# cartographer-project/cartographer

Measured on AMD Instinct MI355X. Metric: candidate poses scored/sec, higher is better.
Workload: dtype u8/int32; 1 GPU; C2: 2D FastCorrelativeScanMatcher MatchFullSubmap (branch and bound): 1000-point scan vs 1 400x400 submap(s) per GPU, depth 7, full-angle search, m...; submaps_per_gpu=1, rotations=2373, found=1

## Files before the change

### cartographer_amd/csrc/cmx_common.h

```cpp
#ifndef CMX_COMMON_H_
#define CMX_COMMON_H_

#include <hip/hip_runtime.h>

#include <cstdarg>
#include <cstdint>
#include <cstdio>
#include <cstring>
#include <functional>
#include <mutex>
#include <string>
#include <vector>

#include "../../include/cartographer_mi355x.h"

namespace cmx {

void SetLastError(const char* fmt, ...);
const char* LastError();

struct HipError {
  cmx_status status;
};

// ... 26 lines not shown
  } catch (const std::bad_alloc&) {
    SetLastError("host allocation failed");
    return CMX_OUT_OF_MEMORY;
  } catch (const std::exception& e) {
    SetLastError("exception: %s", e.what());
    return CMX_DEVICE_ERROR;
  }
}

#define CMX_DEBUG_OPTIONS(X)                                                                      \
  X(rt2d_legacy)                 \
  X(rt2d_tile)                                        \
  X(rt2d_groups)                                   \
  X(rt2d_target)                                    \
  X(rt2d_lds_kb)                                         \
  X(rt2d_no_image_cache)             \
  X(rt2d_parts)                                 \
  X(rt2d_host_par)         \
  X(rt2d_tables_serial)    \
  X(rt2d_first_part)       \
  X(rt2d_image_kernels)    \
  X(rt2d_no_lane)          \
  X(rt2d_parts_pool)       \
  X(rt2d_grid_share)       \
  X(rt2d_unfused)            \
  X(rt2d_no_bounds)        \
  X(rt2d_bounds)           \
  X(rt2d_bounds_fused)     \
  X(rt2d_bounds_level)     \
  X(rt2d_bounds_verify)    \
  X(rt2d_tsdf_batch_legacy)  \
  X(rt2d_tsdf_batch_bulk)  \
  X(rt2d_tsdf_verify)      \
  X(timeline)                  \
  X(trace)                       \
  X(host_trace)                          \
  X(launch_serial)         \
  X(sync)                      \
  X(no_copy_kernels)             \
  X(timing)                \
  X(no_direct_results)     \
  X(frontier_capacity)     \
  X(comm_virtual_ranks)    \
  X(comm_force_rccl)       \
  X(fast2d_unfused)                    \
  X(fast2d_store_scans)                   \
  X(fast2d_fused_threads)                            \
  X(fast2d_fanout)         \
  X(fast2d_group)          \
  X(fast2d_group_verify)   \
  X(fast2d_levels_per_stage)                                    \
  X(fast2d_wave_levels)                        \
  X(fast2d_xcd_affinity)                          \
  X(fast2d_queue)          \
  X(fast2d_queue_blocks)                \
  X(fast2d_queue_capacity)              \
  X(fast2d_queue_lost)       \
  X(filters_generic)       \
  X(fast3d_byte_loads)                             \
  X(fast3d_affinity)                              \
  X(fast3d_no_families)                             \
  X(fast3d_no_oct)                                         \
  X(fast3d_batch)                                                 \
  X(fast3d_chunk_cells)    \
  X(rt3d_legacy)                  \
  X(rt3d_no_tiles)                      \
  X(rt3d_verify)                  \
  X(rt3d_no_rotblocks)              \
  X(rt3d_rotblock_permille)  \
  X(rt3d_crosscheck)           \
  X(rt3d_expand_all)       \
  X(rt3d_unstaged)                                     \
  X(rt3d_no_boxes)                            \
  X(rt3d_report)                                             \
  X(rt3d_segments)                         \
  X(rt3d_group_rotations)                                  \
  X(rt3d_group_tile_kb)                                   \
  X(rt3d_group_float)                          \
  X(rt3d_cand_threads)                                   \
  X(rt3d_cand_rotations)                                    \
  X(rt3d_cand_tile_kb)
struct DebugOptions {
#define CMX_DEBUG_FIELD(name) int name = 0;
  CMX_DEBUG_OPTIONS(CMX_DEBUG_FIELD)
#undef CMX_DEBUG_FIELD
};
const DebugOptions& Debug();
bool DebugSet(const char* name, int value);

void UseDevice(int device);

void ParallelFor(int n, int serial_below, const std::function<void(int)>& fn);

class LaunchTurn {
 public:
  LaunchTurn();
  ~LaunchTurn();
  LaunchTurn(const LaunchTurn&) = delete;
  LaunchTurn& operator=(const LaunchTurn&) = delete;
 private:
  bool held_;
};

class HostLane {
 public:
  HostLane();
// ... 161 lines not shown
```

### cartographer_amd/csrc/fast_2d.hip

```cpp
#include <algorithm>
#include <chrono>
#include <cstring>
#include <memory>
#include <type_traits>
#include <utility>

#include "fast_2d_device.h"
#include "fast_2d_internal.h"

namespace cmx {
namespace {

constexpr int kSeedsPerProblem = 64;

constexpr int kMaxStages = kMaxDepth + 2;

constexpr int kCountStride = 32;
constexpr int kQueues = 2048;
struct alignas(8) QueueCtl {
  int head;
  int reserved;
  int pad[30];
};
struct Counters {
// ... 15 lines not shown
  int frontier_overflow;
  int leaf_overflow;
  unsigned wave_gathers;
  int pad;
  unsigned queue_stats[8];
};

struct NodeList {
  Node2D* nodes;
  int* counts;
  int sub_capacity;
};

__device__ __forceinline__ int ListReserve(const NodeList& list, int sub, int m) {
  return atomicAdd(&list.counts[sub * kCountStride], m);
}
__device__ __forceinline__ bool ListStore(const NodeList& list, int sub, int slot,
                                          const Node2D& nd) {
  if (slot >= list.sub_capacity) return false;
  list.nodes[static_cast<size_t>(sub) * list.sub_capacity + slot] = nd;
  return true;
}
__device__ __forceinline__ int ListMaxCount(const NodeList& list) {
  const int lane = threadIdx.x & 63;
  return WaveMax(min(list.counts[lane * kCountStride], list.sub_capacity));
}

__device__ __forceinline__ int NodeProblem(const Node2D& nd) { return nd.problem & 0xffffff; }
__device__ __forceinline__ int NodeLevel(const Node2D& nd) { return nd.problem >> 24; }

__device__ __forceinline__ Node2D CoarseNode(const Fast2DProblem& P, int problem, int s,
                                             int local) {
  const int2 dims = P.coarse_dims[s];
  const int4 bd = P.bounds[s];
  const int step = 1 << (P.depth - 1);
  const int ix = local / dims.y, iy = local - ix * dims.y;
  const int c = s * P.coarse_stride + local;
  Node2D nd;
  nd.problem = problem | ((P.depth - 1) << 24);
  nd.scan = s;
  nd.dx = bd.x + ix * step;
  nd.dy = bd.z + iy * step;
  nd.score = P.coarse_score[c];
  nd.coarse_index = c;
  nd.path = 0;
  nd.coarse_score = nd.score;
  return nd;
}

struct SeedScratch {
  int hist[1024];
  int wave_total[4];
  int threshold_bin;
  int found_scan;
  int total;
};

__device__ __forceinline__ bool PickSeed(const Fast2DProblem& P, int n, int want,
                                         SeedScratch* sh, int* scan_out) {
  const int tid = threadIdx.x, lane = tid & 63, T = blockDim.x;
  for (int i = tid; i < 1024; i += T) sh->hist[i] = 0;
  if (tid == 0) { sh->found_scan = -1; sh->total = 0; }
  __syncthreads();
  const int S = P.num_scans;
  const long long range = 255ll * n + 1;
  const auto* scan_best = AsGlobal(P.scan_best);
  const auto* coarse_dims = AsGlobal(P.coarse_dims);
  const bool grouped = P.group > 1;
  const auto best_of = [&](int s) -> int {
    if (grouped) {
      const int first = s - s % kFusedGroup;
      if (s != first + (S - first >= kFusedGroup ? 1 : 0)) return -1;
    }
    return scan_best[s].x;
  };
  constexpr int kOwn = 16;
  int own[kOwn];
#pragma unroll
  for (int k = 0; k < kOwn; ++k) {
    const int s = tid + k * T;
    own[k] = s < S ? best_of(s) : -1;
  }
  int total = 0;
#pragma unroll
  for (int k = 0; k < kOwn; ++k)
    if (own[k] >= 0) atomicAdd(&sh->hist[static_cast<int>(own[k] * 1024ll / range)], 1);
  for (int s = tid + kOwn * T; s < S; s += T) {
    const int b = best_of(s);
    if (b >= 0) atomicAdd(&sh->hist[static_cast<int>(b * 1024ll / range)], 1);
  }
  if (want == 0) {
    for (int s = tid; s < S; s += T) total += coarse_dims[s].x * coarse_dims[s].y;
    total = WaveSum(total);
    if (lane == 0 && total) atomicAdd(&sh->total, total);
  }
  __syncthreads();
  if (tid < 64) {
    int mine = 0;
#pragma unroll
    for (int k = 0; k < 16; ++k) mine += sh->hist[1023 - 16 * lane - k];
    int incl = mine;
#pragma unroll
    for (int off = 1; off < 64; off <<= 1) {
      const int o = __shfl_up(incl, off, 64);
      if (lane >= off) incl += o;
    }
    const unsigned long long reached = __ballot(incl >= kSeedsPerProblem);
    int tb = 0;
    if (reached) {
      const int first = __ffsll(static_cast<long long>(reached)) - 1;
      if (lane == first) {
        int acc = incl - mine;
        for (int k = 0; k < 16; ++k) {
          const int b = 1023 - 16 * lane - k;
          acc += sh->hist[b];
          if (acc >= kSeedsPerProblem) { tb = b; break; }
        }
        sh->threshold_bin = tb;
      }
    } else if (lane == 0) {
      sh->threshold_bin = 0;
    }
  }
  __syncthreads();
  const int tb = sh->threshold_bin;
  const auto qualifies = [&](int best) {
    return best >= 0 && static_cast<int>(best * 1024ll / range) >= tb &&
           ToScore(P, best, n) > P.min_score;
  };
  int count = 0;
#pragma unroll
  for (int k = 0; k < kOwn; ++k) count += qualifies(own[k]) ? 1 : 0;
  for (int s = tid + kOwn * T; s < S; s += T) count += qualifies(best_of(s)) ? 1 : 0;
  int incl = count;
#pragma unroll
  for (int off = 1; off < 64; off <<= 1) {
    const int o = __shfl_up(incl, off, 64);
    if (lane >= off) incl += o;
  }
  if (lane == 63) sh->wave_total[tid >> 6] = incl;
  __syncthreads();
  int before = incl - count;
  for (int w = 0; w < (tid >> 6); ++w) before += sh->wave_total[w];
  if (want >= before && want < before + count) {
    int k = before, found = -1;
#pragma unroll
    for (int j = 0; j < kOwn; ++j) {
      if (found < 0 && qualifies(own[j])) {
        if (k == want) found = tid + j * T;
        ++k;
      }
    }
    for (int s = tid + kOwn * T; s < S && found < 0; s += T) {
      if (!qualifies(best_of(s))) continue;
      if (k == want) found = s;
      ++k;
    }
    sh->found_scan = found;
  }
  __syncthreads();
  *scan_out = sh->found_scan;
  return sh->found_scan >= 0;
}

constexpr int kPointCache = 4096;

struct BlockContext {
  LevelDesc level[kMaxDepth];
  uint32_t cache[kPointCache];
  const uint32_t* global_pts;
  float min_s, score_scale, min_score;
  int n, cached;
  int max_x, max_y;
};

__device__ __forceinline__ void LoadContext(const Fast2DProblem& P, int n, int scan,
                                            BlockContext* ctx, bool stored = false) {
  const uint32_t* pts = P.discrete + static_cast<size_t>(scan) * n;
  const bool cached = n <= kPointCache;
  if (P.recompute_scans && !stored) {
    const float2 rot = P.scan_rot[scan];
    for (int i = threadIdx.x; i < n; i += blockDim.x) ctx->cache[i] = ScanCell(P, rot, i);
  } else if (cached) {
    const auto* gp = AsGlobal(pts);
    for (int i = threadIdx.x; i < n; i += blockDim.x) ctx->cache[i] = gp[i];
  }
  if (threadIdx.x < kMaxDepth && static_cast<int>(threadIdx.x) < P.depth)
    ctx->level[threadIdx.x] = P.level[threadIdx.x];
  if (threadIdx.x == 64) {
    const int4 bd = P.bounds[scan];
    ctx->max_x = bd.y;
    ctx->max_y = bd.w;
    ctx->global_pts = pts;
    ctx->cached = cached;
    ctx->n = n;
    ctx->min_s = P.min_s;
    ctx->score_scale = P.score_scale;
    ctx->min_score = P.min_score;
  }
  __syncthreads();
}

__device__ __forceinline__ float ToScoreCtx(const BlockContext& ctx, int sum) {
  return ctx.min_s + (static_cast<float>(sum) / static_cast<float>(ctx.n)) * ctx.score_scale;
}

struct ChildScratch {
  int partial[4][4];
  float child_score[4];
  int rank[4];
  int nvalid;
};

__device__ __forceinline__ void ScoreChildren(const BlockContext& ctx, int dx, int dy,
                                              int child_level, ChildScratch* sh) {
// ... 773 lines not shown
                                        int home, Node2D* out, unsigned* lost_races,
                                        unsigned* slot_rereads) {
  for (;;) {
    const unsigned long long hr =
        LoadAgent(reinterpret_cast<const unsigned long long*>(&counters->queue[home].head));
    const int head = static_cast<int>(hr & 0xffffffffu);
    const int reserved = min(static_cast<int>(hr >> 32), Q.capacity);
    if (reserved <= head) return false;
    if (TakeSlot(counters, home, head)) {
      ReadSlot(Q, home, head, out, slot_rereads);
      return true;
    }
    ++*lost_races;
  }
}

__device__ __forceinline__ bool Steal(const TreeQueue& Q, Counters* __restrict__ counters,
                                      int home, int queues, unsigned salt, int windows,
                                      int max_lost, Node2D* out, unsigned* lost_races,
                                      unsigned* slot_rereads) {
  const int lane = threadIdx.x & 63;
  int lost = 0;
  for (int w = 0; w < windows; ++w) {
    const int base = static_cast<int>((static_cast<unsigned>(home) * 2654435761u + salt * 40503u + w * 64u) %
                                      static_cast<unsigned>(queues));
    const int mine = (base + lane) % queues;
    const unsigned long long hr =
        LoadAgent(reinterpret_cast<const unsigned long long*>(&counters->queue[mine].head));
    const int head = static_cast<int>(hr & 0xffffffffu);
    const int reserved = min(static_cast<int>(hr >> 32), Q.capacity);
    const unsigned long long avail = __ballot(reserved > head);
    if (avail == 0) continue;
    int skip = static_cast<int>((salt + home) % static_cast<unsigned>(__popcll(avail)));
    unsigned long long rest = avail;
    while (skip-- > 0) rest &= rest - 1;
    const int l = __ffsll(static_cast<long long>(rest)) - 1;
    const int q = (base + l) % queues;
    const int slot = __builtin_amdgcn_readlane(head, l);
    if (TakeSlot(counters, q, slot)) {
      ReadSlot(Q, q, slot, out, slot_rereads);
      return true;
    }
    ++*lost_races;
    if (++lost >= max_lost) return false;
    --w;
    ++salt;
  }
  return false;
}

constexpr int kChainCells = 16;
constexpr uint32_t kNoCell = 0x80008000u;

__device__ __forceinline__ void RecordLeafAgent(const Node2D& leaf, const NodeList& leaves,
                                                int sub, Counters* __restrict__ counters) {
  const int slot = ListReserve(leaves, sub, 1);
  if (slot >= leaves.sub_capacity) {
    __hip_atomic_store(&counters->leaf_overflow, 1, __ATOMIC_RELAXED, __HIP_MEMORY_SCOPE_AGENT);
    return;
  }
  unsigned long long v[4];
  __builtin_memcpy(v, &leaf, sizeof(Node2D));
  unsigned long long* at = reinterpret_cast<unsigned long long*>(
      &leaves.nodes[static_cast<size_t>(sub) * leaves.sub_capacity + slot]);
#pragma unroll
  for (int k = 0; k < 4; ++k)
    __hip_atomic_store(&at[k], v[k], __ATOMIC_RELAXED, __HIP_MEMORY_SCOPE_AGENT);
}

__global__ void __launch_bounds__(256)
TreeQueueKernel(const Fast2DProblem* __restrict__ problems, ProblemState* __restrict__ states, int n,
                NodeList in, TreeQueue Q, NodeList leaves, Counters* __restrict__ counters,
                SelectState* __restrict__ sel, BestLeaf* __restrict__ best_out, int num_problems,
                ProblemState* __restrict__ states_out, CountersSummary* __restrict__ summary,
                const unsigned* __restrict__ tail_dev, unsigned* __restrict__ tail_host,
                int tail_words, int counters_trace, int max_lost) {
  static_assert(sizeof(Node2D) == 32, "a node is eight words: eight granules, four leaf stores");
  const int lane = threadIdx.x & 63;
  const int wave_id = blockIdx.x * 4 + __builtin_amdgcn_readfirstlane(threadIdx.x >> 6);
  const int num_waves = gridDim.x * 4;
  const int queues = min(num_waves, kQueues);
  const int home = wave_id % queues;
  unsigned steals = 0;
  unsigned long long scored = 0, expanded = 0;
  unsigned gathers = 0;
  unsigned q_pops = 0, q_lost = 0, q_rereads = 0, q_pushed = 0, q_listed = 0, q_chains = 0;
  int stat_problem = -1;
  const auto flush_stats = [&]() {
    if (lane == 0 && stat_problem >= 0 && expanded) {
      ProblemState& st = states[stat_problem];
      atomicAdd(&st.scored_shard[wave_id & (kStatShards - 1)], scored);
      atomicAdd(&st.expanded_shard[wave_id & (kStatShards - 1)], expanded);
    }
    scored = expanded = 0;
  };
  const int in_slots = ListMaxCount(in) * kSubLists;
  int round = 0;
  Node2D mine{};
  unsigned mine_bits = 0;
  bool round_loaded = false, share_done = false;
  bool pushed_any = false;
  Node2D nd;
  for (;;) {
    bool have = false;
    while (!have && !share_done) {
      if (!round_loaded) {
        if (wave_id + static_cast<long long>(round) * 64 * num_waves >= in_slots) { share_done = true; break; }
        const long long i = wave_id + (static_cast<long long>(round) * 64 + lane) * num_waves;
        ++round;
        mine_bits = 0;
        if (i < in_slots) {
          const int in_sub = static_cast<int>(i & (kSubLists - 1)), j = static_cast<int>(i / kSubLists);
          if (j < min(in.counts[in_sub * kCountStride], in.sub_capacity)) {
            mine = in.nodes[static_cast<size_t>(in_sub) * in.sub_capacity + j];
            mine_bits = max(__float_as_uint(fmaxf(mine.score, 0.f)), 1u);
          }
        }
        round_loaded = true;
      }
      const unsigned top = static_cast<unsigned>(WaveMax(static_cast<int>(mine_bits)));
      const float bound_now = __uint_as_float(LoadAgent(&states[0].best_bits));
      if (top == 0 || (num_problems == 1 && __uint_as_float(top) < bound_now)) {
        round_loaded = false;
        continue;
      }
      const int l = __ffsll(static_cast<long long>(__ballot(mine_bits == top))) - 1;
      nd.problem = __builtin_amdgcn_readlane(mine.problem, l);
      nd.scan = __builtin_amdgcn_readlane(mine.scan, l);
      nd.dx = __builtin_amdgcn_readlane(mine.dx, l);
      nd.dy = __builtin_amdgcn_readlane(mine.dy, l);
      nd.score = __uint_as_float(__builtin_amdgcn_readlane(__float_as_uint(mine.score), l));
      nd.coarse_index = __builtin_amdgcn_readlane(mine.coarse_index, l);
      nd.path = __builtin_amdgcn_readlane(mine.path, l);
      nd.coarse_score =
          __uint_as_float(__builtin_amdgcn_readlane(__float_as_uint(mine.coarse_score), l));
      if (lane == l) mine_bits = 0;
      have = true;
      ++q_listed;
    }
    if (!have) {
      if (!(pushed_any && PopHome(Q, counters, home, &nd, &q_lost, &q_rereads)) &&
          !Steal(Q, counters, home, queues, ++steals, 2, max_lost, &nd, &q_lost, &q_rereads))
        break;
      ++q_pops;
    }
    const int problem = __builtin_amdgcn_readfirstlane(NodeProblem(nd));
    const Fast2DProblem& P = problems[problem];
    ProblemState& st = states[problem];
    float best = __uint_as_float(LoadAgent(&st.best_bits));
    if (nd.score < best) continue;
    if (problem != stat_problem) { flush_stats(); stat_problem = problem; }
    ++q_chains;
    const auto* pts = AsGlobal(P.discrete) + static_cast<size_t>(nd.scan) * n;
    uint32_t cell[kChainCells];
#pragma unroll
    for (int j = 0; j < kChainCells; ++j) {
      const int i = j * kWave + lane;
      cell[j] = kNoCell;
      if (j * kWave < n) cell[j] = i < n ? pts[i] : kNoCell;
    }
    const int4 bd = P.bounds[nd.scan];
    const float min_score = P.min_score;
    for (;;) {
      const int child_level = __builtin_amdgcn_readfirstlane(NodeLevel(nd) - 1);
      const LevelDesc& Lm = P.level[child_level];
      const int half = 1 << child_level;
      const int ndx = __builtin_amdgcn_readfirstlane(nd.dx), ndy = __builtin_amdgcn_readfirstlane(nd.dy);
      const bool vx = ndx + half <= bd.y, vy = ndy + half <= bd.w;
      const int ax = ndx + 2 * half - 1, ay = ndy + 2 * half - 1;
      const int parent_ub = SumUpperBound(P, nd.score, n);
      struct { int qx, qy, qtx; } L;
      L.qx = __builtin_amdgcn_readfirstlane(Lm.qx);
      L.qy = __builtin_amdgcn_readfirstlane(Lm.qy);
      L.qtx = __builtin_amdgcn_readfirstlane(Lm.qtx);
      const unsigned long long quads_address = reinterpret_cast<unsigned long long>(Lm.quads);
      const unsigned long long quads_uniform =
          static_cast<unsigned long long>(static_cast<unsigned>(
              __builtin_amdgcn_readfirstlane(static_cast<unsigned>(quads_address)))) |
          (static_cast<unsigned long long>(static_cast<unsigned>(
               __builtin_amdgcn_readfirstlane(static_cast<unsigned>(quads_address >> 32)))) << 32);
      const unsigned long long quad_bytes =
          static_cast<unsigned long long>((L.qy + 3) >> 2) * static_cast<unsigned>(L.qtx) * 128ull;
      const __amdgpu_buffer_rsrc_t quad_rsrc = __builtin_amdgcn_make_buffer_rsrc(
          reinterpret_cast<uint32_t*>(quads_uniform), 0, static_cast<int>(quad_bytes), 0x00020000);
      typedef unsigned short Halves __attribute__((ext_vector_type(2)));
      uint32_t even = 0, odd = 0;
      int seen_max = 0;
      bool dead = false;
      const auto gather = [&](auto first_tag, auto count_tag) {
        constexpr int kFirst = decltype(first_tag)::value, kCount = decltype(count_tag)::value;
        uint32_t v[kCount];
#pragma unroll
        for (int u = 0; u < kCount; ++u) {
          const uint32_t p = cell[kFirst + u];
          const unsigned X = static_cast<unsigned>(static_cast<short>(p & 0xffffu) + ax);
          const unsigned Y = static_cast<unsigned>(static_cast<short>(p >> 16) + ay);
          const bool inside = X < static_cast<unsigned>(L.qx) && Y < static_cast<unsigned>(L.qy);
          const unsigned tile = __umul24(Y >> 2, static_cast<unsigned>(L.qtx)) + (X >> 3);
          const unsigned byte = (tile << 7) | ((Y & 3u) << 5) | ((X & 7u) << 2);
          v[u] = __builtin_amdgcn_raw_buffer_load_b32(quad_rsrc, inside ? byte : 0xfffffff0u, 0, 0);
        }
#pragma unroll
        for (int u = 0; u < kCount; ++u) {
          const uint32_t e = v[u] & 0x00ff00ffu, o = (v[u] >> 8) & 0x00ff00ffu;
          even += e;
          odd += o;
          Halves eh, oh;
          __builtin_memcpy(&eh, &e, 4);
          __builtin_memcpy(&oh, &o, 4);
          const Halves m = __builtin_elementwise_max(eh, oh);
          seen_max += static_cast<int>(max(m.x, m.y));
        }
      };
      gather(std::integral_constant<int, 0>{}, std::integral_constant<int, 4>{});
      gathers += 4;
      if (n > 4 * kWave) {
        const int most = static_cast<int>(max(max(even & 0xffffu, even >> 16),
                                              max(odd & 0xffffu, odd >> 16)));
        if (ToScore(P, parent_ub - WaveSum(seen_max - most), n) < best) {
          dead = true;
        } else {
          if (n > 8 * kWave) {
            gather(std::integral_constant<int, 4>{}, std::integral_constant<int, 12>{});
            gathers += 12;
          } else {
            gather(std::integral_constant<int, 4>{}, std::integral_constant<int, 4>{});
            gathers += 4;
          }
        }
      }
      ++expanded;
      scored += (1 + (vx ? 1 : 0)) * (1 + (vy ? 1 : 0));
      if (dead) break;
      const int total[4] = {WaveSum(static_cast<int>(even & 0xffffu)), WaveSum(static_cast<int>(odd & 0xffffu)),
                            WaveSum(static_cast<int>(even >> 16)), WaveSum(static_cast<int>(odd >> 16))};
      float sc[4];
#pragma unroll
      for (int k = 0; k < 4; ++k) {
        const bool valid = ((k >> 1) == 0 || vx) && ((k & 1) == 0 || vy);
        sc[k] = valid ? ToScore(P, total[k], n) : -1.f;
      }
      const int k = lane & 3;
      const float mine = k == 0 ? sc[0] : (k == 1 ? sc[1] : (k == 2 ? sc[2] : sc[3]));
      int rank = 0;
#pragma unroll
      for (int o = 0; o < 4; ++o)
        if (o != k && sc[o] >= 0.f && (sc[o] > mine || (sc[o] == mine && o < k))) ++rank;
      best = fmaxf(best, __uint_as_float(LoadAgent(&st.best_bits)));
      const bool keep = lane < 4 && mine >= 0.f && mine >= best;
      const int kbest = __ffsll(static_cast<long long>(__ballot(lane < 4 && mine >= 0.f && rank == 0))) - 1;
      Node2D child;
      child.problem = problem | (child_level << 24);
      child.scan = nd.scan;
      child.dx = nd.dx + (k >> 1) * half;
      child.dy = nd.dy + (k & 1) * half;
      child.score = mine;
      child.coarse_index = nd.coarse_index;
      child.path = nd.path | (static_cast<unsigned>(rank) << (2 * child_level));
      child.coarse_score = nd.coarse_score;
      const bool best_kept = (__ballot(keep) >> kbest) & 1ull;
      if (child_level == 0) {
        if (best_kept && lane == kbest && child.score > min_score) {
          RecordLeafAgent(child, leaves, wave_id & (kSubLists - 1), counters);
          atomicMax(&st.best_bits, __float_as_uint(child.score));
        }
// ... 167 lines not shown

SearchRun::SearchRun(Workspace& ws, const PreparedBatch& batch, BatchResult* result)
    : ws(ws), batch(batch), result(result), num(batch.num_problems), n(batch.n),
      depth(batch.h_problems[0].depth) {
  const auto capacity = [](int v, int fallback) {
    return v >= kSubLists ? std::min(v, fallback) / kSubLists * kSubLists : fallback;
  };
  const int frontier_default = static_cast<int>(
      std::min<long long>(1ll << 25, std::max<long long>(1ll << 21, 65536ll * num)));
  frontier_capacity = capacity(Debug().frontier_capacity, frontier_default);
  frontier_sub = frontier_capacity / kSubLists;
  const int leaf_capacity = capacity(0, 1 << 20);
  Node2D* d_leaves = ws.dev[12].ReserveAs<Node2D>(leaf_capacity);
  d_counters = reinterpret_cast<Counters*>(batch.d_misc);
  d_tail = SearchTail(batch.d_misc + sizeof(Counters), num);
  leaf_list = NodeList{d_leaves, d_counters->leaves, leaf_capacity / kSubLists};
  h_tail = SearchTail(static_cast<char*>(ws.pinned[3].Reserve(SearchTail::Bytes(num))), num);
  direct = Debug().no_direct_results == 0 && h_tail.bytes % sizeof(unsigned) == 0;
}

void SearchRun::FetchResults(bool published) {
  if (!published)
    SmallCopyAsync(h_tail.base, d_tail.base, h_tail.bytes, false, ws.stream);
  const auto t0 = std::chrono::steady_clock::now();
  CMX_HIP(hipStreamSynchronize(ws.stream));
  g_host_wait_ns += std::chrono::duration_cast<std::chrono::nanoseconds>(
                        std::chrono::steady_clock::now() - t0).count();
}

void SearchRun::PrepareStrictRetry() {
  CMX_REQUIRE(num_chunks < (1 << 12), "branch-and-bound overflow not resolvable");
  if (h_tail.summary->frontier_overflow) num_chunks *= 4;
  strict = 1;
  for (int p = 0; p < num; ++p) {
    const float floor_score = std::max(batch.h_problems[p].min_score, 0.f);
    unsigned floor_bits;
    std::memcpy(&floor_bits, &floor_score, sizeof(float));
    if (h_tail.states[p].best_bits > floor_bits) h_tail.states[p].best_bits -= 1;
  }
  CMX_HIP(hipMemcpyAsync(batch.d_states, h_tail.states, num * sizeof(ProblemState),
                         hipMemcpyHostToDevice, ws.stream));
  CMX_HIP(hipMemsetAsync(d_counters, 0, sizeof(Counters), ws.stream));
}

void RunDepthOne(SearchRun& run) {
  Workspace& ws = run.ws;
  SelectDepthOneKernel<<<run.num, 1024, 0, ws.stream>>>(
      run.batch.d_problems, run.batch.d_states, run.n, run.d_tail.best, run.d_tail.states);
  CMX_HIP(hipGetLastError());
  RecordEvent(ws.ev_end, ws.stream);
  run.FetchResults(false);
}

bool QueueSearchPossible(const SearchRun& run) {
  bool queue_ok = QueueSearchWanted(run.n, run.num);
  for (const Fast2DProblem& P : run.batch.h_problems) {
    queue_ok = queue_ok && (P.recompute_scans == 0 || P.store_scans != 0);
    for (int l = 0; l + 1 < run.depth; ++l)
      queue_ok = queue_ok && static_cast<unsigned long long>((P.level[l].qy + 3) >> 2) *
                                     static_cast<unsigned>(P.level[l].qtx) * 128ull < (1ull << 31);
  }
  return queue_ok;
}

enum class QueueOutcome { kDone, kLeafOverflow, kQueueOverflow };

QueueOutcome RunQueueSearch(SearchRun& run, std::unique_ptr<LaunchTurn> turn) {
  Workspace& ws = run.ws;
  const PreparedBatch& batch = run.batch;
  BatchResult* result = run.result;
  const int num = run.num, n = run.n;
  const long long wanted = std::max<long long>(1ll << 20, 65536ll * num);
  int sub_capacity = static_cast<int>(std::min<long long>(wanted, 1ll << 23) / kQueues);
  if (Debug().fast2d_queue_capacity > 0) sub_capacity = Debug().fast2d_queue_capacity;
  TreeQueue queue;
  queue.capacity = sub_capacity;
  queue.slots = static_cast<unsigned long long*>(ws.tagged[0].Acquire(
      static_cast<size_t>(kQueues) * sub_capacity * 8 * sizeof(unsigned long long), ws.stream,
      &queue.epoch));
  run.d_front[0] = ws.dev[10].ReserveAs<Node2D>(run.frontier_capacity);
  FilterCoarseKernel<<<dim3(DivUp(batch.max_scans, 4), num), 256, 0, ws.stream>>>(
      batch.d_problems, batch.d_states, n, 0, 1, 0, 0, run.Front(0),
      run.d_counters);
  run.Mark("filter");
  RecordEvent(ws.ev_x0, ws.stream);
  const int blocks = Debug().fast2d_queue_blocks > 0
                         ? Debug().fast2d_queue_blocks
                         : std::min(2048, 256 * std::max(1, (num + 3) / 4));
  TreeQueueKernel<<<blocks, 256, 0, ws.stream>>>(
      batch.d_problems, batch.d_states, n, run.Front(0), queue, run.leaf_list, run.d_counters,
      run.d_tail.sel, run.d_tail.best, num, run.d_tail.states, run.d_tail.summary,
      run.d_tail.words(), run.PublishTo(), run.h_tail.num_words(),
      batch.trace && batch.trace->enabled() ? 1 : 0,
      Debug().fast2d_queue_lost > 0 ? Debug().fast2d_queue_lost : 3);
  run.Mark("queue");
  CMX_HIP(hipGetLastError());
  RecordEvent(ws.ev_x1, ws.stream);
  result->expansion_launches = 1;
  RecordEvent(ws.ev_end, ws.stream);
  turn.reset();
  run.FetchResults(run.direct);
  const CountersSummary& h_counters = *run.h_tail.summary;
  result->expansion_lookups = 64ll * h_counters.wave_gathers;
  for (int p = 0; p < num; ++p)
    for (int k = 0; k < kStatShards; ++k)
      result->expansion_nodes += run.h_tail.states[p].expanded_shard[k];
  if (h_counters.leaf_overflow) return QueueOutcome::kLeafOverflow;
  if (h_counters.frontier_overflow) return QueueOutcome::kQueueOverflow;
  return QueueOutcome::kDone;
}

void RunLevelSynchronous(SearchRun& run) {
  Workspace& ws = run.ws;
  const PreparedBatch& batch = run.batch;
// ... 47 lines not shown
        run.d_counters, run.d_tail.summary, run.d_tail.words(), run.PublishTo(),
        run.h_tail.num_words());
    run.Mark("select");
    CMX_HIP(hipGetLastError());
    RecordEvent(ws.ev_end, ws.stream);
    run.FetchResults(run.direct);
    if (!strict) {
      for (int st = 0; st < result->expansion_launches; ++st)
        result->expansion_nodes += h_counters.frontier_total[st];
      result->expansion_lookups = 64ll * h_counters.wave_gathers;
    }
    if (!h_counters.frontier_overflow && !h_counters.leaf_overflow) break;
    run.PrepareStrictRetry();
  }
}

void TraceListSizes(const CountersSummary& h_counters) {
  fprintf(stderr, "[cmx trace] list sizes:");
  for (int st = 0; st < kMaxStages; ++st)
    if (h_counters.frontier_total[st])
      fprintf(stderr, " frontier[%d]=%d", st, h_counters.frontier_total[st]);
  long long leaves = 0;
  for (int k = 0; k < kSubLists; ++k) leaves += h_counters.leaves[k];
  fprintf(stderr, " leaves=%lld\n", leaves);
  const unsigned* q = h_counters.queue_stats;
  if (q[5])
    fprintf(stderr, "[cmx trace] work queue: %u chains (%u nodes from the list, %u popped), %u "
            "pushed, %u lost races, %u slot re-reads\n", q[5], q[4], q[0], q[3], q[1], q[2]);
}

}

bool QueueSearchWanted(int n, int num) {
  return Debug().fast2d_queue != 2 && n <= kChainCells * kWave && (num < 4 || Debug().fast2d_queue == 1);
}

void ReserveSearchScratch(Workspace& ws, int num, PreparedBatch* batch) {
  batch->d_misc = static_cast<char*>(ws.dev[14].Reserve(SearchMiscBytes(num)));
  batch->num_counter_words = static_cast<int>(sizeof(Counters) / sizeof(int));
}

thread_local long long g_host_wait_ns = 0;

void RunBranchAndBound(Workspace& ws, const PreparedBatch& batch, BatchResult* result) {
  const int num = batch.num_problems;
  const int depth = batch.h_problems[0].depth;
  for (const Fast2DProblem& P : batch.h_problems)
    CMX_REQUIRE(P.depth == depth, "all matchers of a batch must share branch_and_bound_depth");
  SearchRun run(ws, batch, result);
  if (depth == 1) {
    RunDepthOne(run);
  } else {
    std::unique_ptr<LaunchTurn> turn(new LaunchTurn);
    DiveKernel<<<dim3(kSeedsPerProblem * (batch.any_group ? kFusedGroup : 1), num), 256, 0, ws.stream>>>(
        batch.d_problems, batch.d_states, run.n, run.leaf_list, run.d_counters);
    run.Mark("seed+dive");
    bool searched = false;
    if (QueueSearchPossible(run)) {
      switch (RunQueueSearch(run, std::move(turn))) {
        case QueueOutcome::kDone:
          searched = true;
          break;
        case QueueOutcome::kLeafOverflow:
          run.PrepareStrictRetry();
          break;
        case QueueOutcome::kQueueOverflow:
          CMX_HIP(hipMemsetAsync(run.d_counters, 0, sizeof(Counters), ws.stream));
          break;
      }
    }
    turn.reset();
    if (!searched) RunLevelSynchronous(run);
  }

  result->best.assign(run.h_tail.best, run.h_tail.best + num);
  result->states.assign(run.h_tail.states, run.h_tail.states + num);
  if (depth > 1) {
    if (batch.trace && batch.trace->enabled()) TraceListSizes(*run.h_tail.summary);
    result->d_leaves = run.leaf_list.nodes;
    result->leaf_sub_capacity = run.leaf_list.sub_capacity;
    result->leaf_counts.assign(run.h_tail.summary->leaves, run.h_tail.summary->leaves + kSubLists);
  }
  result->device_ms = ElapsedMs(ws.ev_begin, ws.ev_end);
  result->dominant_ms = ElapsedMs(ws.ev_k0, ws.ev_k1);
  if (result->expansion_launches > 0) result->expansion_ms = ElapsedMs(ws.ev_x0, ws.ev_x1);
}

}
```

### cartographer_amd/csrc/fast_2d_coarse.hip

```cpp
#include <algorithm>
#include <cmath>
#include <cstring>
#include <memory>
#include <mutex>
#include <vector>

#include "fast_2d_device.h"
#include "fast_2d_internal.h"

namespace cmx {
namespace {

constexpr int kMaxBuckets = 4096;
constexpr int kMaxCoarsePerScan = 4096;
constexpr int kMaxAccCells = 12288;

__global__ void __launch_bounds__(256)
PrepScansKernel(const Fast2DProblem* __restrict__ problems, const float* __restrict__ xyz, int n,
                ProblemState* __restrict__ states, int* __restrict__ counters_words,
                int num_counter_words) {
  if (counters_words)
    for (int i = (blockIdx.y * gridDim.x + blockIdx.x) * blockDim.x + threadIdx.x;
         i < num_counter_words; i += gridDim.x * gridDim.y * blockDim.x)
      counters_words[i] = 0;
// ... 424 lines not shown
      : "v"(base), "n"(o), "n"(o + 2), "n"(o + 16), "n"(o + 18), "n"(o + 32), "n"(o + 34),
        "n"(o + 48), "n"(o + 50), "n"(o + 64), "n"(o + 66), "n"(o + 80), "n"(o + 82),
        "n"(o + 96), "n"(o + 98), "n"(o + 112), "n"(o + 114)
      : "memory");
}

template <bool kTimeline>
__device__ __forceinline__ void FusedPass(const Fast2DProblem& P, ProblemState* state, int n,
                                          int acc_cap, int s0, int timeline_block) {
  extern __shared__ __attribute__((aligned(16))) unsigned char fused_smem[];
  const auto uni = [](int v) { return __builtin_amdgcn_readfirstlane(v); };
  const int n_pad = (n + 63) & ~63;
  const int G = P.group > 1 ? kFusedGroup : 1;
  auto* pts_all = reinterpret_cast<uint32_t*>(fused_smem);
  int* misc = reinterpret_cast<int*>(pts_all + G * n_pad);
  int* cand_acc = misc + kFusedMisc;
  const int T = blockDim.x;
  const int waves = T >> 6;
  const int lane = threadIdx.x & 63;
  const int wave = __builtin_amdgcn_readfirstlane(threadIdx.x >> 6);
  const auto stamp = [&](int k) {
    if constexpr (kTimeline) Stamp(P.timeline, timeline_block, k);
  };
  const int gcount = uni(misc[1]), gm = uni(misc[2]);
  const bool far = uni(misc[7]) != 0;
  const int2 dims_all = make_int2(uni(misc[4]), uni(misc[5]));
  const int PI = P.plane_i, PJ = P.plane_j, PIJ = PI * PJ;
  const int shift = P.depth - 1, w = 1 << shift;
  const unsigned zero_plane = 1u << (2 * (P.depth - 1));
  const int group = lane >> 4, sub = lane & 15;
  const int begin = static_cast<int>(static_cast<long long>(n) * wave / waves);
  const int end = static_cast<int>(static_cast<long long>(n) * (wave + 1) / waves);
  constexpr int kSteps = 16;
  uint32_t* const wave_words = reinterpret_cast<uint32_t*>(cand_acc + acc_cap) + 64 * wave;
  const unsigned group_base = static_cast<unsigned>(reinterpret_cast<uintptr_t>(
      (__attribute__((address_space(3))) uint32_t*)(wave_words + group)));
  int2* const scratch = reinterpret_cast<int2*>(misc + 8);
  const bool verify = (P.group_verify & 1) != 0;
    const bool group_pass = G > 1;
    const int gp = group_pass ? gm : 0;
    const uint32_t* const pts = pts_all + gp * n_pad;
    const int* const mine = misc + 16 + 8 * gp;
    const int4 bd = make_int4(uni(mine[0]), uni(mine[1]), uni(mine[2]), uni(mine[3]));
    const int2 dims = group_pass ? dims_all : make_int2(uni(mine[4]), uni(mine[5]));
    const int lift = group_pass ? kGroupDilation : 0;
    const int pitch = dims.y + 2 * PJ - 2;
    const int BW = dims.x + PI - 1, BH = dims.y + PJ - 1;

  int lane_const[4];
#pragma unroll
  for (int j = 0; j < 4; ++j) {
    const int cell = min(4 * sub + j, PIJ - 1);
    lane_const[j] = (cell % PI + dims.x + PI - 2) * pitch + (cell / PI + dims.y + PJ - 2);
  }
  uint32_t cur = 0;
  uint32_t a0 = 0, a1 = 0, a2 = 0, a3 = 0;
  const auto flush = [&]() {
    const int at = static_cast<int>(cur) - 1;
    if (a0) atomicAdd(&cand_acc[lane_const[0] - at], static_cast<int>(a0));
    if (a1) atomicAdd(&cand_acc[lane_const[1] - at], static_cast<int>(a1));
    if (a2) atomicAdd(&cand_acc[lane_const[2] - at], static_cast<int>(a2));
    if (a3) atomicAdd(&cand_acc[lane_const[3] - at], static_cast<int>(a3));
    a0 = a1 = a2 = a3 = 0;
  };
  const unsigned long long planes_bits =
      reinterpret_cast<unsigned long long>(group_pass ? P.planes_group : P.planes);
  const unsigned planes_lo = static_cast<unsigned>(
      __builtin_amdgcn_readfirstlane(static_cast<int>(static_cast<unsigned>(planes_bits))));
  const unsigned planes_hi = static_cast<unsigned>(
      __builtin_amdgcn_readfirstlane(static_cast<int>(static_cast<unsigned>(planes_bits >> 32))));
  const uint8_t* const planes_uniform = reinterpret_cast<const uint8_t*>(
      (static_cast<unsigned long long>(planes_hi) << 32) | planes_lo);
  const __amdgpu_buffer_rsrc_t rsrc = __builtin_amdgcn_make_buffer_rsrc(
      const_cast<uint8_t*>(planes_uniform), 0, static_cast<int>((zero_plane + 1) * 64), 0x00020000);
  for (int base_i = begin; base_i < end; base_i += 64) {
    const int chunk_index = (base_i - begin) >> 6;
    if constexpr (kTimeline) {
      if (chunk_index == 0) stamp(8);
      else if (chunk_index <= 4) stamp(11 + chunk_index);
    }
    uint32_t my_word = zero_plane;
    if (base_i + lane < end) {
      const uint32_t packed = pts[base_i + lane];
      const int U = static_cast<short>(packed & 0xffffu) + bd.x + w - 1 + lift;
      const int V = static_cast<short>(packed >> 16) + bd.z + w - 1 + lift;
      const int bx = (U >> shift) + dims.x - 1, by = (V >> shift) + dims.y - 1;
      if (bx >= 0 && bx < BW && by >= 0 && by < BH)
        my_word = static_cast<uint32_t>((V & (w - 1)) * w + (U & (w - 1))) |
                  (static_cast<uint32_t>(bx * pitch + by + 1) << 16);
    }
    wave_words[lane] = my_word;
    __builtin_amdgcn_wave_barrier();
    uint32_t block[kSteps];
    uint32_t plane[kSteps];
    uint32_t q[kSteps];
    ReadHalves8<0>(group_base, plane, block);
    ReadHalves8<8>(group_base, plane + 8, block + 8);
#pragma unroll
    for (int k = 0; k < kSteps; ++k)
      q[k] = __builtin_amdgcn_raw_buffer_load_b32(rsrc, (plane[k] << 6) | (4 * sub), 0, 0);
    __builtin_amdgcn_wave_barrier();
    if constexpr (kTimeline) {
      if (chunk_index == 0) {
        stamp(9);
        __builtin_amdgcn_s_waitcnt(0x0f70);
        stamp(10);
// ... 629 lines not shown
```

Measured before the change: 10.16 billion candidates/s.

## Replace block-per-seed dive with wave-per-seed greedy chain dive kernel

Adds DiveWaveKernel, where each 64-lane wave takes one seed (four seeds per 256-thread block) and walks greedily down the levels. It uses the same quad-tile buffer-load gather as the queue chain walker, and the gather and level setup are factored into shared helpers. PickSeeds now selects several seed scans in one histogram pass, which cuts the number of blocks launched and the seed-selection work per block. The old block-wide DiveKernel stays available behind a debug flag. A separate asm barrier pins lane_const in VGPRs in the coarse kernel.

```diff
diff --git a/cartographer_amd/csrc/cmx_common.h b/cartographer_amd/csrc/cmx_common.h
--- a/cartographer_amd/csrc/cmx_common.h
+++ b/cartographer_amd/csrc/cmx_common.h
@@ -102,6 +102,7 @@
   X(fast2d_levels_per_stage)                                    \
   X(fast2d_wave_levels)                        \
   X(fast2d_xcd_affinity)                          \
+  X(fast2d_dive)           \
   X(fast2d_queue)          \
   X(fast2d_queue_blocks)                \
   X(fast2d_queue_capacity)              \
diff --git a/cartographer_amd/csrc/fast_2d.hip b/cartographer_amd/csrc/fast_2d.hip
--- a/cartographer_amd/csrc/fast_2d.hip
+++ b/cartographer_amd/csrc/fast_2d.hip
@@ -91,15 +91,16 @@
   int hist[1024];
   int wave_total[4];
   int threshold_bin;
-  int found_scan;
+  int found_scan[4];
   int total;
 };
 
-__device__ __forceinline__ bool PickSeed(const Fast2DProblem& P, int n, int want,
-                                         SeedScratch* sh, int* scan_out) {
+__device__ __forceinline__ void PickSeeds(const Fast2DProblem& P, int n, int want0, int wants,
+                                          SeedScratch* sh) {
   const int tid = threadIdx.x, lane = tid & 63, T = blockDim.x;
   for (int i = tid; i < 1024; i += T) sh->hist[i] = 0;
-  if (tid == 0) { sh->found_scan = -1; sh->total = 0; }
+  if (tid < 4) sh->found_scan[tid] = -1;
+  if (tid == 0) sh->total = 0;
   __syncthreads();
   const int S = P.num_scans;
   const long long range = 255ll * n + 1;
@@ -128,7 +129,7 @@
     const int b = best_of(s);
     if (b >= 0) atomicAdd(&sh->hist[static_cast<int>(b * 1024ll / range)], 1);
   }
-  if (want == 0) {
+  if (want0 == 0) {
     for (int s = tid; s < S; s += T) total += coarse_dims[s].x * coarse_dims[s].y;
     total = WaveSum(total);
     if (lane == 0 && total) atomicAdd(&sh->total, total);
@@ -181,25 +182,30 @@
   __syncthreads();
   int before = incl - count;
   for (int w = 0; w < (tid >> 6); ++w) before += sh->wave_total[w];
-  if (want >= before && want < before + count) {
-    int k = before, found = -1;
+  const int want_end = want0 + wants;
+  if (want0 < before + count && want_end > before) {
+    int k = before;
 #pragma unroll
     for (int j = 0; j < kOwn; ++j) {
-      if (found < 0 && qualifies(own[j])) {
-        if (k == want) found = tid + j * T;
+      if (qualifies(own[j])) {
+        if (k >= want0 && k < want_end) sh->found_scan[k - want0] = tid + j * T;
         ++k;
       }
     }
-    for (int s = tid + kOwn * T; s < S && found < 0; s += T) {
+    for (int s = tid + kOwn * T; s < S && k < want_end; s += T) {
       if (!qualifies(best_of(s))) continue;
-      if (k == want) found = s;
+      if (k >= want0) sh->found_scan[k - want0] = s;
       ++k;
     }
-    sh->found_scan = found;
-  }
-  __syncthreads();
-  *scan_out = sh->found_scan;
-  return sh->found_scan >= 0;
+  }
+  __syncthreads();
+}
+
+__device__ __forceinline__ bool PickSeed(const Fast2DProblem& P, int n, int want,
+                                         SeedScratch* sh, int* scan_out) {
+  PickSeeds(P, n, want, 1, sh);
+  *scan_out = sh->found_scan[0];
+  return sh->found_scan[0] >= 0;
 }
 
 constexpr int kPointCache = 4096;
@@ -1079,6 +1085,167 @@
 constexpr int kChainCells = 16;
 constexpr uint32_t kNoCell = 0x80008000u;
 
+template <bool kRecompute>
+__device__ __forceinline__ void LoadChainCells(const Fast2DProblem& P, int n, int scan,
+                                               uint32_t (&cell)[kChainCells]) {
+  const int lane = threadIdx.x & 63;
+  const auto* pts = AsGlobal(P.discrete) + static_cast<size_t>(scan) * n;
+  if constexpr (kRecompute) {
+    const float2 rot = P.scan_rot[scan];
+#pragma unroll
+    for (int u = 0; u < kChainCells; ++u) cell[u] = kNoCell;
+#pragma unroll 1
+    for (int j = 0; j * kWave < n; ++j) {
+      const int i = j * kWave + lane;
+      const uint32_t c = i < n ? ScanCell(P, rot, i) : kNoCell;
+#pragma unroll
+      for (int u = 0; u < kChainCells; ++u) cell[u] = u == j ? c : cell[u];
+    }
+  } else {
+#pragma unroll
+    for (int j = 0; j < kChainCells; ++j) {
+      const int i = j * kWave + lane;
+      cell[j] = kNoCell;
+      if (j * kWave < n) cell[j] = i < n ? pts[i] : kNoCell;
+    }
+  }
+}
+
+struct ChainLevel {
+  int qx, qy, qtx;
+  int half;
+  int ax, ay;
+  __amdgpu_buffer_rsrc_t quad_rsrc;
+};
+
+__device__ __forceinline__ ChainLevel MakeChainLevel(const Fast2DProblem& P, int child_level,
+                                                     int dx, int dy) {
+  const LevelDesc& Lm = P.level[child_level];
+  ChainLevel L;
+  L.half = 1 << child_level;
+  L.ax = dx + 2 * L.half - 1;
+  L.ay = dy + 2 * L.half - 1;
+  L.qx = __builtin_amdgcn_readfirstlane(Lm.qx);
+  L.qy = __builtin_amdgcn_readfirstlane(Lm.qy);
+  L.qtx = __builtin_amdgcn_readfirstlane(Lm.qtx);
+  const unsigned long long quads_address = reinterpret_cast<unsigned long long>(Lm.quads);
+  const unsigned long long quads_uniform =
+      static_cast<unsigned long long>(static_cast<unsigned>(
+          __builtin_amdgcn_readfirstlane(static_cast<unsigned>(quads_address)))) |
+      (static_cast<unsigned long long>(static_cast<unsigned>(
+           __builtin_amdgcn_readfirstlane(static_cast<unsigned>(quads_address >> 32)))) << 32);
+  const unsigned long long quad_bytes =
+      static_cast<unsigned long long>((L.qy + 3) >> 2) * static_cast<unsigned>(L.qtx) * 128ull;
+  L.quad_rsrc = __builtin_amdgcn_make_buffer_rsrc(
+      reinterpret_cast<uint32_t*>(quads_uniform), 0, static_cast<int>(quad_bytes), 0x00020000);
+  return L;
+}
+
+template <int kFirst, int kCount, bool kWantMax>
+__device__ __forceinline__ void ChainGather(const ChainLevel& L, const uint32_t (&cell)[kChainCells],
+                                            uint32_t* even, uint32_t* odd, int* seen_max) {
+  typedef unsigned short Halves __attribute__((ext_vector_type(2)));
+  uint32_t v[kCount];
+#pragma unroll
+  for (int u = 0; u < kCount; ++u) {
+    const uint32_t p = cell[kFirst + u];
+    const unsigned X = static_cast<unsigned>(static_cast<short>(p & 0xffffu) + L.ax);
+    const unsigned Y = static_cast<unsigned>(static_cast<short>(p >> 16) + L.ay);
+    const bool inside = X < static_cast<unsigned>(L.qx) && Y < static_cast<unsigned>(L.qy);
+    const unsigned tile = __umul24(Y >> 2, static_cast<unsigned>(L.qtx)) + (X >> 3);
+    const unsigned byte = (tile << 7) | ((Y & 3u) << 5) | ((X & 7u) << 2);
+    v[u] = __builtin_amdgcn_raw_buffer_load_b32(L.quad_rsrc, inside ? byte : 0xfffffff0u, 0, 0);
+  }
+#pragma unroll
+  for (int u = 0; u < kCount; ++u) {
+    const uint32_t e = v[u] & 0x00ff00ffu, o = (v[u] >> 8) & 0x00ff00ffu;
+    *even += e;
+    *odd += o;
+    if constexpr (kWantMax) {
+      Halves eh, oh;
+      __builtin_memcpy(&eh, &e, 4);
+      __builtin_memcpy(&oh, &o, 4);
+      const Halves m = __builtin_elementwise_max(eh, oh);
+      *seen_max += static_cast<int>(max(m.x, m.y));
+    }
+  }
+}
+
+__global__ void __launch_bounds__(256)
+DiveWaveKernel(const Fast2DProblem* __restrict__ problems, ProblemState* __restrict__ states, int n,
+               NodeList leaves, Counters* __restrict__ counters) {
+  const int problem = blockIdx.y;
+  const Fast2DProblem& P = problems[problem];
+  ProblemState& st = states[problem];
+  if (st.error) return;
+  __shared__ SeedScratch seed_scratch;
+  const bool grouped = P.group > 1;
+  const int seeds = grouped ? 1 : 4;
+  const int want0 = static_cast<int>(blockIdx.x) * seeds;
+  if (want0 >= kSeedsPerProblem) return;
+  PickSeeds(P, n, want0, seeds, &seed_scratch);
+  if (blockIdx.x == 0 && threadIdx.x == 0) st.coarse_total = seed_scratch.total;
+  const int lane = threadIdx.x & 63;
+  const int wave = __builtin_amdgcn_readfirstlane(threadIdx.x >> 6);
+  if (grouped && wave >= kFusedGroup) return;
+  int seed_scan = __builtin_amdgcn_readfirstlane(seed_scratch.found_scan[grouped ? 0 : wave]);
+  if (seed_scan < 0) return;
+  if (grouped) {
+    seed_scan = seed_scan - seed_scan % kFusedGroup + wave;
+    if (seed_scan >= P.num_scans) return;
+  }
+  const Node2D seed = CoarseNode(P, problem, seed_scan, P.scan_best[seed_scan].y);
+  uint32_t cell[kChainCells];
+  const bool stored =
+      !P.recompute_scans ||
+      (P.store_scans && !(ToScore(P, P.scan_best[seed_scan].x, n) < fmaxf(P.min_score, 0.f)));
+  if (__builtin_amdgcn_readfirstlane(stored ? 1 : 0)) LoadChainCells<false>(P, n, seed_scan, cell);
+  else LoadChainCells<true>(P, n, seed_scan, cell);
+  const int4 bd = P.bounds[seed_scan];
+  const int depth = P.depth;
+  int dx = __builtin_amdgcn_readfirstlane(seed.dx), dy = __builtin_amdgcn_readfirstlane(seed.dy);
+  float score = seed.score;
+  unsigned long long scored = 0;
+  for (int child_level = depth - 2; child_level >= 0; --child_level) {
+    const ChainLevel L = MakeChainLevel(P, child_level, dx, dy);
+    const bool vx = dx + L.half <= bd.y, vy = dy + L.half <= bd.w;
+    uint32_t even = 0, odd = 0;
+    if (n > 8 * kWave) ChainGather<0, 16, false>(L, cell, &even, &odd, nullptr);
+    else if (n > 4 * kWave) ChainGather<0, 8, false>(L, cell, &even, &odd, nullptr);
+    else ChainGather<0, 4, false>(L, cell, &even, &odd, nullptr);
+    const int total[4] = {WaveSum(static_cast<int>(even & 0xffffu)), WaveSum(static_cast<int>(odd & 0xffffu)),
+                          WaveSum(static_cast<int>(even >> 16)), WaveSum(static_cast<int>(odd >> 16))};
+    int kbest = 0, nvalid = 0;
+    float best_score = -1.f;
+#pragma unroll
+    for (int k = 0; k < 4; ++k) {
+      const bool valid = ((k >> 1) == 0 || vx) && ((k & 1) == 0 || vy);
+      const float sc = valid ? ToScore(P, total[k], n) : -1.f;
+      nvalid += valid ? 1 : 0;
+      if (sc >= 0.f && (k == 0 || sc > best_score)) { kbest = k; best_score = sc; }
+    }
+    kbest = __builtin_amdgcn_readfirstlane(kbest);
+    dx += (kbest >> 1) * L.half;
+    dy += (kbest & 1) * L.half;
+    score = best_score;
+    scored += nvalid;
+  }
+  if (lane == 0) {
+    if (score > P.min_score) {
+      Node2D leaf = seed;
+      leaf.problem = problem;
+      leaf.dx = dx;
+      leaf.dy = dy;
+      leaf.score = score;
+      RecordLeaf(leaf, leaves, counters);
+      atomicMax(&st.best_bits, __float_as_uint(score));
+    }
+    const int shard = (blockIdx.x * 4 + wave) & (kStatShards - 1);
+    atomicAdd(&st.scored_shard[shard], scored);
+    atomicAdd(&st.expanded_shard[shard], static_cast<unsigned long long>(depth - 1));
+  }
+}
+
 __device__ __forceinline__ void RecordLeafAgent(const Node2D& leaf, const NodeList& leaves,
                                                 int sub, Counters* __restrict__ counters) {
   const int slot = ListReserve(leaves, sub, 1);
@@ -1178,66 +1345,23 @@
     if (nd.score < best) continue;
     if (problem != stat_problem) { flush_stats(); stat_problem = problem; }
     ++q_chains;
-    const auto* pts = AsGlobal(P.discrete) + static_cast<size_t>(nd.scan) * n;
     uint32_t cell[kChainCells];
-#pragma unroll
-    for (int j = 0; j < kChainCells; ++j) {
-      const int i = j * kWave + lane;
-      cell[j] = kNoCell;
-      if (j * kWave < n) cell[j] = i < n ? pts[i] : kNoCell;
-    }
+    LoadChainCells<false>(P, n, nd.scan, cell);
     const int4 bd = P.bounds[nd.scan];
     const float min_score = P.min_score;
     for (;;) {
       const int child_level = __builtin_amdgcn_readfirstlane(NodeLevel(nd) - 1);
-      const LevelDesc& Lm = P.level[child_level];
-      const int half = 1 << child_level;
       const int ndx = __builtin_amdgcn_readfirstlane(nd.dx), ndy = __builtin_amdgcn_readfirstlane(nd.dy);
+      const ChainLevel L = MakeChainLevel(P, child_level, ndx, ndy);
+      const int half = L.half;
       const bool vx = ndx + half <= bd.y, vy = ndy + half <= bd.w;
-      const int ax = ndx + 2 * half - 1, ay = ndy + 2 * half - 1;
       const int parent_ub = SumUpperBound(P, nd.score, n);
-      struct { int qx, qy, qtx; } L;
-      L.qx = __builtin_amdgcn_readfirstlane(Lm.qx);
-      L.qy = __builtin_amdgcn_readfirstlane(Lm.qy);
-      L.qtx = __builtin_amdgcn_readfirstlane(Lm.qtx);
-      const unsigned long long quads_address = reinterpret_cast<unsigned long long>(Lm.quads);
-      const unsigned long long quads_uniform =
-          static_cast<unsigned long long>(static_cast<unsigned>(
-              __builtin_amdgcn_readfirstlane(static_cast<unsigned>(quads_address)))) |
-          (static_cast<unsigned long long>(static_cast<unsigned>(
-               __builtin_amdgcn_readfirstlane(static_cast<unsigned>(quads_address >> 32)))) << 32);
-      const unsigned long long quad_bytes =
-          static_cast<unsigned long long>((L.qy + 3) >> 2) * static_cast<unsigned>(L.qtx) * 128ull;
-      const __amdgpu_buffer_rsrc_t quad_rsrc = __builtin_amdgcn_make_buffer_rsrc(
-          reinterpret_cast<uint32_t*>(quads_uniform), 0, static_cast<int>(quad_bytes), 0x00020000);
-      typedef unsigned short Halves __attribute__((ext_vector_type(2)));
       uint32_t even = 0, odd = 0;
       int seen_max = 0;
       bool dead = false;
       const auto gather = [&](auto first_tag, auto count_tag) {
-        constexpr int kFirst = decltype(first_tag)::value, kCount = decltype(count_tag)::value;
-        uint32_t v[kCount];
-#pragma unroll
-        for (int u = 0; u < kCount; ++u) {
-          const uint32_t p = cell[kFirst + u];
-          const unsigned X = static_cast<unsigned>(static_cast<short>(p & 0xffffu) + ax);
-          const unsigned Y = static_cast<unsigned>(static_cast<short>(p >> 16) + ay);
-          const bool inside = X < static_cast<unsigned>(L.qx) && Y < static_cast<unsigned>(L.qy);
-          const unsigned tile = __umul24(Y >> 2, static_cast<unsigned>(L.qtx)) + (X >> 3);
-          const unsigned byte = (tile << 7) | ((Y & 3u) << 5) | ((X & 7u) << 2);
-          v[u] = __builtin_amdgcn_raw_buffer_load_b32(quad_rsrc, inside ? byte : 0xfffffff0u, 0, 0);
-        }
-#pragma unroll
-        for (int u = 0; u < kCount; ++u) {
-          const uint32_t e = v[u] & 0x00ff00ffu, o = (v[u] >> 8) & 0x00ff00ffu;
-          even += e;
-          odd += o;
-          Halves eh, oh;
-          __builtin_memcpy(&eh, &e, 4);
-          __builtin_memcpy(&oh, &o, 4);
-          const Halves m = __builtin_elementwise_max(eh, oh);
-          seen_max += static_cast<int>(max(m.x, m.y));
-        }
+        ChainGather<decltype(first_tag)::value, decltype(count_tag)::value, true>(L, cell, &even,
+                                                                                  &odd, &seen_max);
       };
       gather(std::integral_constant<int, 0>{}, std::integral_constant<int, 4>{});
       gathers += 4;
@@ -1511,14 +1635,19 @@
   run.FetchResults(false);
 }
 
+bool ChainWalkPossible(const SearchRun& run) {
+  bool chain_ok = run.n <= kChainCells * kWave;
+  for (const Fast2DProblem& P : run.batch.h_problems)
+    for (int l = 0; l + 1 < run.depth; ++l)
+      chain_ok = chain_ok && static_cast<unsigned long long>((P.level[l].qy + 3) >> 2) *
+                                     static_cast<unsigned>(P.level[l].qtx) * 128ull < (1ull << 31);
+  return chain_ok;
+}
+
 bool QueueSearchPossible(const SearchRun& run) {
-  bool queue_ok = QueueSearchWanted(run.n, run.num);
-  for (const Fast2DProblem& P : run.batch.h_problems) {
+  bool queue_ok = QueueSearchWanted(run.n, run.num) && ChainWalkPossible(run);
+  for (const Fast2DProblem& P : run.batch.h_problems)
     queue_ok = queue_ok && (P.recompute_scans == 0 || P.store_scans != 0);
-    for (int l = 0; l + 1 < run.depth; ++l)
-      queue_ok = queue_ok && static_cast<unsigned long long>((P.level[l].qy + 3) >> 2) *
-                                     static_cast<unsigned>(P.level[l].qtx) * 128ull < (1ull << 31);
-  }
   return queue_ok;
 }
 
@@ -1672,8 +1801,14 @@
     RunDepthOne(run);
   } else {
     std::unique_ptr<LaunchTurn> turn(new LaunchTurn);
-    DiveKernel<<<dim3(kSeedsPerProblem * (batch.any_group ? kFusedGroup : 1), num), 256, 0, ws.stream>>>(
-        batch.d_problems, batch.d_states, run.n, run.leaf_list, run.d_counters);
+    if (Debug().fast2d_dive != 1 && ChainWalkPossible(run)) {
+      DiveWaveKernel<<<dim3(batch.any_group ? kSeedsPerProblem : kSeedsPerProblem / 4, num), 256, 0,
+                       ws.stream>>>(batch.d_problems, batch.d_states, run.n, run.leaf_list,
+                                    run.d_counters);
+    } else {
+      DiveKernel<<<dim3(kSeedsPerProblem * (batch.any_group ? kFusedGroup : 1), num), 256, 0, ws.stream>>>(
+          batch.d_problems, batch.d_states, run.n, run.leaf_list, run.d_counters);
+    }
     run.Mark("seed+dive");
     bool searched = false;
     if (QueueSearchPossible(run)) {
diff --git a/cartographer_amd/csrc/fast_2d_coarse.hip b/cartographer_amd/csrc/fast_2d_coarse.hip
--- a/cartographer_amd/csrc/fast_2d_coarse.hip
+++ b/cartographer_amd/csrc/fast_2d_coarse.hip
@@ -500,6 +500,7 @@
   for (int j = 0; j < 4; ++j) {
     const int cell = min(4 * sub + j, PIJ - 1);
     lane_const[j] = (cell % PI + dims.x + PI - 2) * pitch + (cell / PI + dims.y + PJ - 2);
+    asm volatile("" : "+v"(lane_const[j]));
   }
   uint32_t cur = 0;
   uint32_t a0 = 0, a1 = 0, a2 = 0, a3 = 0;
```

Measured after the change: 10.86 billion candidates/s, median of 6. 1.07x the previous value.
